# Developer-Zer0/GIF-synthesis-with-Discrete-Diffusion

Measured on NVIDIA B200. Metric: reverse_step_token_updates_per_sec, higher is better.
Workload: dtype f32

## Files before the change

### gif-synthesis-with-discrete-diffusion_b200/csrc/d3pm_ptx.cuh

```cuda
#pragma once

#include <cuda_runtime.h>
#include <stdint.h>

namespace d3pm {

__device__ __forceinline__ uint32_t smem_u32(const void* p) { return static_cast<uint32_t>(__cvta_generic_to_shared(p)); }

__device__ __forceinline__ void mbar_init(unsigned long long* bar, uint32_t count) {
  asm volatile("mbarrier.init.shared::cta.b64 [%0], %1;" ::"r"(smem_u32(bar)), "r"(count) : "memory");
}
__device__ __forceinline__ void fence_mbarrier_init() { asm volatile("fence.mbarrier_init.release.cluster;" ::: "memory"); }
__device__ __forceinline__ void mbar_expect_tx(unsigned long long* bar, uint32_t bytes) {
  asm volatile("mbarrier.arrive.expect_tx.shared::cta.b64 _, [%0], %1;" ::"r"(smem_u32(bar)), "r"(bytes) : "memory");
}
__device__ __forceinline__ void mbar_arrive(unsigned long long* bar) {
  asm volatile("mbarrier.arrive.shared::cta.b64 _, [%0];" ::"r"(smem_u32(bar)) : "memory");
}
__device__ __forceinline__ void mbar_arrive_remote(unsigned long long* bar, uint32_t cta) {
  uint32_t r;
  asm volatile("mapa.shared::cluster.u32 %0, %1, %2;" : "=r"(r) : "r"(smem_u32(bar)), "r"(cta));
  asm volatile("mbarrier.arrive.release.cluster.shared::cluster.b64 _, [%0];" ::"r"(r) : "memory");
}
__device__ __forceinline__ bool mbar_test(unsigned long long* bar, uint32_t parity) {
  uint32_t done;
  asm volatile(
      "{\n\t.reg .pred p;\n\t"
      "mbarrier.test_wait.parity.shared::cta.b64 p, [%1], %2;\n\t"
      "selp.u32 %0, 1, 0, p;\n\t}"
      : "=r"(done)
      : "r"(smem_u32(bar)), "r"(parity)
      : "memory");
  return done != 0;
}
__device__ __forceinline__ void mbar_wait(unsigned long long* bar, uint32_t parity) {
  asm volatile(
      "{\n\t.reg .pred p;\n\t"
      "WAIT_%=:\n\t"
      "mbarrier.try_wait.parity.shared::cta.b64 p, [%0], %1, %2;\n\t"
      "@p bra DONE_%=;\n\t"
      "bra WAIT_%=;\n\t"
      "DONE_%=:\n\t}"
      ::"r"(smem_u32(bar)), "r"(parity), "r"(0x989680)
      : "memory");
}
__device__ __forceinline__ void mbar_wait_spin(unsigned long long* bar, uint32_t parity) {
  const uint32_t addr = smem_u32(bar);
  uint32_t done;
  do {
    asm volatile(
        "{\n\t.reg .pred p;\n\t"
        "mbarrier.try_wait.parity.shared::cta.b64 p, [%1], %2;\n\t"
        "selp.u32 %0, 1, 0, p;\n\t}"
        : "=r"(done)
        : "r"(addr), "r"(parity)
        : "memory");
  } while (!done);
}
__device__ __forceinline__ void mbar_wait_cluster(unsigned long long* bar, uint32_t parity) {
  asm volatile(
      "{\n\t.reg .pred p;\n\t"
      "WAIT_%=:\n\t"
      "mbarrier.try_wait.parity.acquire.cluster.shared::cta.b64 p, [%0], %1, %2;\n\t"
      "@p bra DONE_%=;\n\t"
      "bra WAIT_%=;\n\t"
      "DONE_%=:\n\t}"
      ::"r"(smem_u32(bar)), "r"(parity), "r"(0x989680)
      : "memory");
}

__device__ __forceinline__ void tma_load(void* dst, const void* src, uint32_t bytes, unsigned long long* bar) {
  asm volatile(
      "cp.async.bulk.shared::cluster.global.mbarrier::complete_tx::bytes [%0], [%1], %2, [%3];"
      ::"r"(smem_u32(dst)), "l"(src), "r"(bytes), "r"(smem_u32(bar))
      : "memory");
}
__device__ __forceinline__ void fence_proxy_async() { asm volatile("fence.proxy.async.shared::cta;" ::: "memory"); }

__device__ __forceinline__ void tc_fence_before() { asm volatile("tcgen05.fence::before_thread_sync;" ::: "memory"); }
__device__ __forceinline__ void tc_fence_after() { asm volatile("tcgen05.fence::after_thread_sync;" ::: "memory"); }
__device__ __forceinline__ void tc_commit(unsigned long long* bar) {
  asm volatile("tcgen05.commit.cta_group::1.mbarrier::arrive::one.shared::cluster.b64 [%0];" ::"r"(smem_u32(bar)) : "memory");
}
__device__ __forceinline__ void tc_commit_pair(unsigned long long* bar) {
  asm volatile("tcgen05.commit.cta_group::2.mbarrier::arrive::one.shared::cluster.multicast::cluster.b64 [%0], %1;" ::"r"(smem_u32(bar)),
               "h"(static_cast<unsigned short>(3))
               : "memory");
}
constexpr uint32_t idesc_tf32(int M, int N) {
  return (1u << 4) | (2u << 7) | (2u << 10) | ((static_cast<uint32_t>(N) >> 3) << 17) | ((static_cast<uint32_t>(M) >> 4) << 24);
}
__device__ __forceinline__ void tc_mma_tf32(uint32_t d_tmem, uint64_t a_desc, uint64_t b_desc, uint32_t idesc, uint32_t accumulate) {
  asm volatile(
      "{\n\t.reg .pred p;\n\t"
      "setp.ne.b32 p, %4, 0;\n\t"
      "tcgen05.mma.cta_group::1.kind::tf32 [%0], %1, %2, %3, p;\n\t}"
      ::"r"(d_tmem), "l"(a_desc), "l"(b_desc), "r"(idesc), "r"(accumulate)
      : "memory");
}
__device__ __forceinline__ void tc_mma_tf32_pair(uint32_t d_tmem, uint64_t a_desc, uint64_t b_desc, uint32_t idesc, uint32_t accumulate) {
  asm volatile(
      "{\n\t.reg .pred p;\n\t"
      "setp.ne.b32 p, %4, 0;\n\t"
      "tcgen05.mma.cta_group::2.kind::tf32 [%0], %1, %2, %3, p;\n\t}"
      ::"r"(d_tmem), "l"(a_desc), "l"(b_desc), "r"(idesc), "r"(accumulate)
      : "memory");
}
__device__ __forceinline__ uint64_t smem_desc(uint32_t addr) {
  return static_cast<uint64_t>((addr >> 4) & 0x3fffu) | (static_cast<uint64_t>(1024 >> 4) << 32) | (1ull << 46) | (2ull << 61);
}

template <int CTAS, int NCOLS>
__device__ __forceinline__ void tmem_alloc(uint32_t* slot) {
  static_assert(CTAS == 1 || CTAS == 2, "cta_group::1 or ::2");
  if constexpr (CTAS == 2)
    asm volatile("tcgen05.alloc.cta_group::2.sync.aligned.shared::cta.b32 [%0], %1;" ::"r"(smem_u32(slot)), "n"(NCOLS) : "memory");
  else
    asm volatile("tcgen05.alloc.cta_group::1.sync.aligned.shared::cta.b32 [%0], %1;" ::"r"(smem_u32(slot)), "n"(NCOLS) : "memory");
}
template <int CTAS>
__device__ __forceinline__ void tmem_relinquish() {
  static_assert(CTAS == 1 || CTAS == 2, "cta_group::1 or ::2");
  if constexpr (CTAS == 2) asm volatile("tcgen05.relinquish_alloc_permit.cta_group::2.sync.aligned;" ::: "memory");
  else asm volatile("tcgen05.relinquish_alloc_permit.cta_group::1.sync.aligned;" ::: "memory");
}
template <int CTAS, int NCOLS>
__device__ __forceinline__ void tmem_dealloc(uint32_t taddr) {
  static_assert(CTAS == 1 || CTAS == 2, "cta_group::1 or ::2");
  if constexpr (CTAS == 2) asm volatile("tcgen05.dealloc.cta_group::2.sync.aligned.b32 %0, %1;" ::"r"(taddr), "n"(NCOLS) : "memory");
  else asm volatile("tcgen05.dealloc.cta_group::1.sync.aligned.b32 %0, %1;" ::"r"(taddr), "n"(NCOLS) : "memory");
}
__device__ __forceinline__ void tmem_ld16(uint32_t taddr, uint32_t (&v)[16]) {
  asm volatile(
      "tcgen05.ld.sync.aligned.32x32b.x16.b32 "
      "{%0, %1, %2, %3, %4, %5, %6, %7, %8, %9, %10, %11, %12, %13, %14, %15}, [%16];"
      : "=r"(v[0]), "=r"(v[1]), "=r"(v[2]), "=r"(v[3]), "=r"(v[4]), "=r"(v[5]), "=r"(v[6]), "=r"(v[7]), "=r"(v[8]),
        "=r"(v[9]), "=r"(v[10]), "=r"(v[11]), "=r"(v[12]), "=r"(v[13]), "=r"(v[14]), "=r"(v[15])
      : "r"(taddr)
      : "memory");
}
__device__ __forceinline__ void tmem_ld32(uint32_t taddr, uint32_t (&v)[32]) {
  asm volatile(
      "tcgen05.ld.sync.aligned.32x32b.x32.b32 "
      "{%0, %1, %2, %3, %4, %5, %6, %7, %8, %9, %10, %11, %12, %13, %14, %15, "
      "%16, %17, %18, %19, %20, %21, %22, %23, %24, %25, %26, %27, %28, %29, %30, %31}, [%32];"
      : "=r"(v[0]), "=r"(v[1]), "=r"(v[2]), "=r"(v[3]), "=r"(v[4]), "=r"(v[5]), "=r"(v[6]), "=r"(v[7]), "=r"(v[8]),
        "=r"(v[9]), "=r"(v[10]), "=r"(v[11]), "=r"(v[12]), "=r"(v[13]), "=r"(v[14]), "=r"(v[15]), "=r"(v[16]),
        "=r"(v[17]), "=r"(v[18]), "=r"(v[19]), "=r"(v[20]), "=r"(v[21]), "=r"(v[22]), "=r"(v[23]), "=r"(v[24]),
        "=r"(v[25]), "=r"(v[26]), "=r"(v[27]), "=r"(v[28]), "=r"(v[29]), "=r"(v[30]), "=r"(v[31])
      : "r"(taddr)
      : "memory");
}
__device__ __forceinline__ void tmem_ld_wait() { asm volatile("tcgen05.wait::ld.sync.aligned;" ::: "memory"); }

__device__ __forceinline__ uint32_t cluster_ctarank() {
  uint32_t r;
  asm volatile("mov.u32 %0, %%cluster_ctarank;" : "=r"(r));
  return r;
}
__device__ __forceinline__ void cluster_sync() {
  asm volatile("barrier.cluster.arrive.release;" ::: "memory");
  asm volatile("barrier.cluster.wait.acquire;" ::: "memory");
}

}
```

### gif-synthesis-with-discrete-diffusion_b200/csrc/d3pm_step_stream.cuh

```cuda
#pragma once

#include <cuda_fp16.h>

#include <type_traits>

#include "d3pm_host.h"
#include "d3pm_ptx.cuh"
#include "d3pm_step_rows.cuh"

namespace d3pm {

constexpr int kGroupThreads = 128;
constexpr int kGroupWarps = kGroupThreads / 32;
constexpr int kGroupsPerCta = 4;
constexpr int kStreamThreads = kGroupThreads * kGroupsPerCta;
constexpr int kCandPerRow = 30;
constexpr float kStreamThin = 8.0f;
constexpr float kRedoThin = 16.0f;
constexpr int kCoefSmemRows = 256;
struct RowInfo {
  float A, Bc, Pj, PK, accept;
  uint32_t j;
  int32_t rel;
  int32_t pad;
};

template <int NP, int CPT, bool HAS_U>
struct StreamShape {
  static_assert(CPT == 8 || (CPT == 16 && !HAS_U), "64 classes per thread only fit in registers without the second tensor");
  static constexpr int K = 1024 * NP;
  static constexpr int GT = 256 * NP / CPT;
  static constexpr int NW = GT / 32;
  static constexpr int NG = kStreamThreads / GT;
  static constexpr int SB = 128 / NG;
  static constexpr int RC = 8192 / NG;
  static constexpr int PS = 128 / GT;
  static constexpr int NCALL = CPT / 2;
  static_assert(GT >= 32 && GT <= 128 && NG <= 16, "unsupported group shape");
};

template <int NP, int CPT, bool HAS_U>
struct __align__(128) GroupSmem {
  using Sh = StreamShape<NP, CPT, HAS_U>;
  float c[1024 * NP];
  float u[HAS_U ? 1024 * NP : 4];
  alignas(16) float red[3][6 * 4];
  unsigned long long full;
  unsigned long long keys[4];
  uint32_t redo_cnt;
  uint32_t pad;
  RowInfo info[Sh::SB];
  uint32_t cand_cnt[Sh::SB];
  uint32_t cand_k[Sh::SB][kCandPerRow];
  float cand_p[Sh::SB][kCandPerRow];
  int32_t redo[Sh::RC];
};

__device__ __forceinline__ void group_bar(int id) {
  asm volatile("bar.sync %0, %1;" ::"r"(id), "n"(kGroupThreads) : "memory");
}
struct GroupSync {
  int id;
  __device__ __forceinline__ void operator()() const { group_bar(id); }
};
template <int NW>
struct StreamSync {
  int id;
  __device__ __forceinline__ void operator()() const {
    if (NW == 1) __syncwarp();
    else asm volatile("bar.sync %0, %1;" ::"r"(id), "n"(32 * NW) : "memory");
  }
};
__device__ __forceinline__ float4 lds4(const float* p) { return *reinterpret_cast<const float4*>(p); }
template <int LD>
struct LogitType {
  static constexpr uint32_t kBytes = LD == D3PM_LOGITS_F32 ? 4u : 2u;
  static __device__ __forceinline__ float2 widen(uint32_t pair) {
    if constexpr (LD == D3PM_LOGITS_BF16) {
      return make_float2(__uint_as_float(pair << 16), __uint_as_float(pair & 0xffff0000u));
    } else {
      return __half22float2(*reinterpret_cast<const __half2*>(&pair));
    }
  }
  static __device__ __forceinline__ void chunk(const float* stage, int q, float2& lo, float2& hi) {
    if constexpr (LD == D3PM_LOGITS_F32) {
      const float4 a = lds4(stage + 4 * q);
      lo = make_float2(a.x, a.y), hi = make_float2(a.z, a.w);
    } else {
      const uint2 raw = *reinterpret_cast<const uint2*>(reinterpret_cast<const unsigned char*>(stage) + 8 * q);
      lo = widen(raw.x), hi = widen(raw.y);
    }
  }
  static __device__ __forceinline__ float one(const float* stage, uint32_t k) {
    if constexpr (LD == D3PM_LOGITS_F32) {
      return stage[k];
    } else {
      const uint32_t h = reinterpret_cast<const unsigned short*>(stage)[k];
      if constexpr (LD == D3PM_LOGITS_BF16) return __uint_as_float(h << 16);
      else return __half2float(__ushort_as_half(static_cast<unsigned short>(h)));
    }
  }
  static __device__ __forceinline__ const void* row(const float* base, unsigned long long elements) {
    return reinterpret_cast<const unsigned char*>(base) + elements * kBytes;
  }
};
template <int NW>
__device__ __forceinline__ float4 lds_warps(const float* p, float neutral) {
  if (NW == 4) return lds4(p);
  const float2 a = *reinterpret_cast<const float2*>(p);
  return make_float4(a.x, a.y, neutral, neutral);
}
template <int NW, int NV, typename Sync>
__device__ __forceinline__ void stream_max_sum(float (&m)[NV], float (&s)[NV], float* scratch, Sync sync) {
  const int lane = threadIdx.x & 31, warp = (threadIdx.x >> 5) & (NW - 1);
#pragma unroll
  for (int v = 0; v < NV; ++v) {
    const float mw = warp_max(m[v]);
    const float mw2 = to_log2_units(mw);
    const float sw = warp_sum(s[v] * ex2(to_log2_units(m[v]) - mw2));
    if (NW == 1) {
      m[v] = mw, s[v] = sw;
    } else if (lane == 0) {
      scratch[(3 * v) * 4 + warp] = mw;
      scratch[(3 * v + 1) * 4 + warp] = mw2;
      scratch[(3 * v + 2) * 4 + warp] = sw;
    }
  }
  sync();
  if constexpr (NW > 1) {
#pragma unroll
  for (int v = 0; v < NV; ++v) {
    const float4 mw = lds_warps<NW>(scratch + (3 * v) * 4, -CUDART_INF_F), mw2 = lds_warps<NW>(scratch + (3 * v + 1) * 4, 0.f);
    const float4 sw = lds_warps<NW>(scratch + (3 * v + 2) * 4, 0.f);
    if (NW == 4) {
      const float M = fmaxf(fmaxf(mw.x, mw.y), fmaxf(mw.z, mw.w));
      const float M2 = to_log2_units(M);
      m[v] = M;
      s[v] = fmaf(sw.x, ex2(mw2.x - M2), fmaf(sw.y, ex2(mw2.y - M2), fmaf(sw.z, ex2(mw2.z - M2), sw.w * ex2(mw2.w - M2))));
    } else {
      const float M = fmaxf(mw.x, mw.y);
      const float M2 = to_log2_units(M);
      m[v] = M;
      s[v] = fmaf(sw.x, ex2(mw2.x - M2), sw.y * ex2(mw2.y - M2));
    }
  }
  }
}

__device__ __forceinline__ float warp_min(float x) {
  float m;
  asm volatile("redux.sync.min.f32 %0, %1, 0xffffffff;" : "=f"(m) : "f"(x));
  return m;
}

template <int NW, int NV, typename Sync>
__device__ __forceinline__ void stream_max(float* mx, float* scratch, Sync sync) {
  const int lane = threadIdx.x & 31, warp = (threadIdx.x >> 5) & (NW - 1);
#pragma unroll
  for (int v = 0; v < NV; ++v) {
    const float a = warp_max(mx[v]);
    if (NW == 1) mx[v] = a;
    else if (lane == 0) scratch[v * 4 + warp] = a;
  }
  sync();
  if constexpr (NW > 1) {
#pragma unroll
  for (int v = 0; v < NV; ++v) {
    const float4 a = lds_warps<NW>(scratch + v * 4, -CUDART_INF_F);
    mx[v] = fmaxf(fmaxf(a.x, a.y), fmaxf(a.z, a.w));
  }
  }
}

template <int NW, int NV, typename Sync>
__device__ __forceinline__ void stream_sum(float (&s)[NV], float* scratch, Sync sync) {
  const int lane = threadIdx.x & 31, warp = (threadIdx.x >> 5) & (NW - 1);
#pragma unroll
  for (int v = 0; v < NV; ++v) {
    const float sw = warp_sum(s[v]);
    if (NW == 1) s[v] = sw;
    else if (lane == 0) scratch[v * 4 + warp] = sw;
  }
  sync();
  if constexpr (NW > 1) {
#pragma unroll
  for (int v = 0; v < NV; ++v) {
    const float4 a = lds_warps<NW>(scratch + v * 4, 0.f);
    s[v] = (a.x + a.y) + (a.z + a.w);
  }
  }
}

template <int NW, typename Sync>
__device__ __forceinline__ unsigned long long stream_max_u64(unsigned long long key, unsigned long long* scratch, Sync sync) {
  const int lane = threadIdx.x & 31, warp = (threadIdx.x >> 5) & (NW - 1);
  key = warp_max_u64(key);
  if (NW == 1) {
    sync();
    return key;
  }
  if (lane == 0) scratch[warp] = key;
  sync();
  unsigned long long best = scratch[0];
#pragma unroll
  for (int w = 1; w < NW; ++w) best = scratch[w] > best ? scratch[w] : best;
  return best;
}

template <int NP, int CPT, bool HAS_U>
__device__ __noinline__ void score_batch(GroupSmem<NP, CPT, HAS_U>& S, int nslots, const ParamNoiseStream& rng, const StepParams& p, int G,
                                         int first_row) {
  using Sh = StreamShape<NP, CPT, HAS_U>;
  constexpr uint32_t K = 1024u * NP;
  const int lane = threadIdx.x & 31, warp = (threadIdx.x >> 5) & (Sh::NW - 1);
  const int sub = lane & 15;
  for (int slot = 2 * warp + (lane >> 4); slot - (lane >> 4) < nslots; slot += 2 * Sh::NW) {
    unsigned long long key = 0ull;
    float lp = 0.f;
    const bool live = slot < nslots;
    RowInfo ri;
    ri.accept = 0.f, ri.rel = 0;
    uint32_t cnt = 0;
    if (live) {
      ri = S.info[slot];
      cnt = S.cand_cnt[slot];
      const uint32_t n = cnt < static_cast<uint32_t>(kCandPerRow) ? cnt : static_cast<uint32_t>(kCandPerRow);
      const uint64_t grow = static_cast<uint64_t>(p.row_offset + (first_row + ri.rel * G));
      for (uint32_t item = static_cast<uint32_t>(sub); item < n + 2u; item += 16u) {
        uint32_t k = 0;
        float P = 0.f;
        bool have = false;
        if (item < n) {
          k = S.cand_k[slot][item];
          const float pe = fminf(fmaxf(S.cand_p[slot][item], kPFloor), 1.0f);
          P = fmaf(pe, ri.A, ri.Bc);
          have = (k != ri.j);
        } else if (item == n) {
          k = K, P = ri.PK, have = true;
        } else if (ri.j != K) {
          k = ri.j, P = ri.Pj, have = true;
        }
        if (have) {
          const float lpk = log_prob_clamped(P);
          const float sc = lpk + gumbel_from_uniform(uniform_from_draw(rng.draw(k, grow)));
          const unsigned long long kk = pack_key(sc, k);
          if (kk > key) key = kk, lp = lpk;
        }
      }
    }
    const unsigned long long mine = key;
#pragma unroll
    for (int o = 8; o > 0; o >>= 1) {
      const unsigned long long other = __shfl_xor_sync(0xffffffffu, key, o);
      key = other > key ? other : key;
    }
    const bool accepted = live && cnt <= static_cast<uint32_t>(kCandPerRow) && key_score(key) >= ri.accept;
    if (live && sub == 0) {
      if (accepted) {
        p.x_prev[first_row + ri.rel * G] = key_class(key);
      } else {
        S.redo[atomicAdd(&S.redo_cnt, 1u)] = ri.rel;
      }
      S.cand_cnt[slot] = 0;
    }
    if (p.winner_post != nullptr && accepted && mine == key && mine != 0ull) p.winner_post[first_row + ri.rel * G] = lp;
  }
}

template <int NP, int CPT, bool HAS_U, bool RECON, int LD = D3PM_LOGITS_F32>
__global__ void __launch_bounds__(kStreamThreads, 1) step_stream_kernel(const __grid_constant__ StepParams p) {
  extern __shared__ __align__(128) unsigned char smem_raw[];
  using Sh = StreamShape<NP, CPT, HAS_U>;
  using Smem = GroupSmem<NP, CPT, HAS_U>;
  constexpr int K = Sh::K, GT = Sh::GT, NW = Sh::NW, NG = Sh::NG, PS = Sh::PS, NCALL = Sh::NCALL;
  constexpr int NC = CPT;
  using LT = LogitType<LD>;
  constexpr uint32_t kRowBytes = K * LT::kBytes;
  uint32_t tid;
  asm volatile("mov.u32 %0, %%tid.x;" : "=r"(tid));
  const int g = tid / GT;
  const int tg = tid % GT;
  Smem& S = reinterpret_cast<Smem*>(smem_raw)[g];
  const StreamSync<NW> sync{g + 1};
  const int G = static_cast<int>(gridDim.x) * NG;
  const int first_row = g * static_cast<int>(gridDim.x) + static_cast<int>(blockIdx.x);
  const int rows = static_cast<int>(p.rows);
  const uint32_t pitch = static_cast<uint32_t>(p.pitch_logits);
  const bool exact_mode = (p.sample_mode == D3PM_SAMPLE_PHILOX_EXACT);
  if (tg == 0) {
    mbar_init(&S.full, 1);
    fence_mbarrier_init();
    S.redo_cnt = 0;
    if (!exact_mode && first_row < rows) {
      const unsigned long long at = static_cast<unsigned long long>(static_cast<uint32_t>(first_row)) * pitch;
      mbar_expect_tx(&S.full, HAS_U ? 2 * kRowBytes : kRowBytes);
      tma_load(S.c, LT::row(p.logits_c, at), kRowBytes, &S.full);
      if (HAS_U) tma_load(S.u, LT::row(p.logits_u, at), kRowBytes, &S.full);
    }
  }
  float* coef_s = reinterpret_cast<float*>(smem_raw + sizeof(Smem) * NG);
  const bool coef_in_smem = p.T <= kCoefSmemRows;
  if (coef_in_smem) {
    for (int i = tid; i < p.T * 16; i += kStreamThreads)
      coef_s[i] = __ldg(p.coef_table + static_cast<size_t>(i >> 4) * D3PM_COEF_STRIDE + (i & 15));
  }
  const ParamNoiseStream rng(NoiseKeysParam(p.keys), p.offset);
  const float thin_c = p.thin_factor > 0.f ? p.thin_factor : kStreamThin;
  for (int i = tg; i < Sh::SB; i += GT) S.cand_cnt[i] = 0;
  __syncthreads();

  auto issue_row = [&](int row) {
    const unsigned long long at = static_cast<unsigned long long>(static_cast<uint32_t>(row)) * pitch;
    fence_proxy_async();
    mbar_expect_tx(&S.full, HAS_U ? 2 * kRowBytes : kRowBytes);
    tma_load(S.c, LT::row(p.logits_c, at), kRowBytes, &S.full);
    if (HAS_U) tma_load(S.u, LT::row(p.logits_u, at), kRowBytes, &S.full);
  };
  auto slot_lo = [](int c) { return (c / PS) * 2 * PS + (c % PS); };

  uint32_t phase = 0;
  uint32_t status_bits = 0;
#ifdef D3PM_STREAM_TIMING
  auto now_ns = [] { unsigned long long v; asm volatile("mov.u64 %0, %%globaltimer;" : "=l"(v)); return v; };
  const unsigned long long tm_start = now_ns();
  unsigned long long tm_main = 0;
  uint32_t tm_rows = 0, tm_redo = 0;
#endif

  auto process_row = [&](auto exact_c, int row, int next_row, uint32_t j, int tt, int slot, int rel) {
    constexpr bool exact = decltype(exact_c)::value;
    const bool masked = (j == static_cast<uint32_t>(K));
    mbar_wait_spin(&S.full, phase);
    phase ^= 1u;

    float2 x[NC][2], z[HAS_U ? NC : 1][2];
#pragma unroll
    for (int i = 0; i < NC; ++i) {
      const int q = GT * i + tg;
      LT::chunk(S.c, q, x[i][0], x[i][1]);
      if (HAS_U) LT::chunk(S.u, q, z[i][0], z[i][1]);
    }
    auto e_of = [&](int i, int h) -> float2& {
      if constexpr (HAS_U) return z[i][h];
      else return x[i][h];
    };
    const float xj = masked ? 0.f : LT::one(S.c, j);
    const float zj = (HAS_U && !masked) ? LT::one(S.u, j) : 0.f;

    float am[2] = {0.f, 0.f};
    if (HAS_U) {
      am[0] = fmaxf(fmaxf(fabsf(x[0][0].x), fabsf(x[0][0].y)), fmaxf(fabsf(x[0][1].x), fabsf(x[0][1].y)));
      am[1] = fmaxf(fmaxf(fabsf(z[0][0].x), fabsf(z[0][0].y)), fmaxf(fabsf(z[0][1].x), fabsf(z[0][1].y)));
    }
#pragma unroll
    for (int i = 1; i < NC; ++i) {
      if (HAS_U)
        am[0] = fmaxf(fmaxf(am[0], fabsf(x[i][0].x)), fmaxf(fabsf(x[i][0].y), fmaxf(fabsf(x[i][1].x), fabsf(x[i][1].y))));
      if (HAS_U)
        am[1] = fmaxf(fmaxf(am[1], fabsf(z[i][0].x)), fmaxf(fabsf(z[i][0].y), fmaxf(fabsf(z[i][1].x), fabsf(z[i][1].y))));
    }
    if (HAS_U) stream_max<NW, 2>(am, S.red[0], sync);
    else sync();
    if (!exact && tg == 0 && next_row >= 0) issue_row(next_row);

    const uint64_t grow = static_cast<uint64_t>(p.row_offset + row);

    float My2, rSy, r, yj;
    const float2 l2e = make_float2(kLog2e, kLog2e);
    if (HAS_U) {
      const float gs = p.guidance_scale, og = 1.0f - gs;
      const float2 gs2 = make_float2(gs, gs), og2 = make_float2(og, og);
      float my = -CUDART_INF_F;
      constexpr float kLnK = NP == 4 ? 8.3178f : (NP == 2 ? 7.6247f : 6.9315f);
      constexpr float kSafeAbs = 0.5f * (69.99f - kLnK);
      const bool no_clamp = (am[0] <= kSafeAbs) && (am[1] <= kSafeAbs) && (fabsf(gs) * am[0] + fabsf(og) * am[1] <= 160.0f);
      if (no_clamp) {
#pragma unroll
        for (int i = 0; i < NC; ++i)
#pragma unroll
          for (int h = 0; h < 2; ++h) {
            const float2 y = __ffma2_rn(gs2, x[i][h], __fmul2_rn(og2, z[i][h]));
            x[i][h] = y;
            my = fmaxf(my, fmaxf(y.x, y.y));
          }
        yj = fmaf(gs, xj, og * zj);
      } else {
        float mx[2], s[2];
        mx[0] = fmaxf(fmaxf(x[0][0].x, x[0][0].y), fmaxf(x[0][1].x, x[0][1].y));
        mx[1] = fmaxf(fmaxf(z[0][0].x, z[0][0].y), fmaxf(z[0][1].x, z[0][1].y));
#pragma unroll
        for (int i = 1; i < NC; ++i) {
          mx[0] = fmaxf(fmaxf(mx[0], x[i][0].x), fmaxf(x[i][0].y, fmaxf(x[i][1].x, x[i][1].y)));
          mx[1] = fmaxf(fmaxf(mx[1], z[i][0].x), fmaxf(z[i][0].y, fmaxf(z[i][1].x, z[i][1].y)));
        }
        stream_max<NW, 2>(mx, S.red[2], sync);
        mx[0] = fmaxf(mx[0], -3.0e38f), mx[1] = fmaxf(mx[1], -3.0e38f);
        {
          const float mc2 = to_log2_units(mx[0]), mu2 = to_log2_units(mx[1]);
          const float2 nmc = make_float2(-mc2, -mc2), nmu = make_float2(-mu2, -mu2);
          float2 sc[2] = {make_float2(0.f, 0.f), make_float2(0.f, 0.f)}, su[2] = {sc[0], sc[0]};
#pragma unroll
          for (int i = 0; i < NC; ++i)
#pragma unroll
            for (int h = 0; h < 2; ++h) {
              const float2 ac = __ffma2_rn(x[i][h], l2e, nmc), au = __ffma2_rn(z[i][h], l2e, nmu);
              sc[h] = __fadd2_rn(sc[h], make_float2(ex2(ac.x), ex2(ac.y)));
              su[h] = __fadd2_rn(su[h], make_float2(ex2(au.x), ex2(au.y)));
            }
          s[0] = (sc[0].x + sc[0].y) + (sc[1].x + sc[1].y);
          s[1] = (su[0].x + su[0].y) + (su[1].x + su[1].y);
        }
        stream_sum<NW, 2>(s, S.red[2] + 2 * 4, sync);
        const float lnSc = ln_rel_sum(mx[0], s[0]), lnSu = ln_rel_sum(mx[1], s[1]);
        const float ta = kClampLo + lnSc, tb = kClampLo + lnSu;
        const float C = fmaf(-gs, lnSc, -og * lnSu);
        const float2 nMc = make_float2(-mx[0], -mx[0]), nMu = make_float2(-mx[1], -mx[1]), C2 = make_float2(C, C);
#pragma unroll
        for (int i = 0; i < NC; ++i)
#pragma unroll
          for (int h = 0; h < 2; ++h) {
            float2 a = __fadd2_rn(x[i][h], nMc), b = __fadd2_rn(z[i][h], nMu);
            a.x = fmaxf(a.x, ta), a.y = fmaxf(a.y, ta);
            b.x = fmaxf(b.x, tb), b.y = fmaxf(b.y, tb);
            const float2 y = __ffma2_rn(gs2, a, __ffma2_rn(og2, b, C2));
            x[i][h] = y;
            my = fmaxf(my, fmaxf(y.x, y.y));
          }
        yj = fmaf(gs, fmaxf(xj - mx[0], ta), fmaf(og, fmaxf(zj - mx[1], tb), C));
      }
      const float my2 = to_log2_units(my);
      {
        const float2 nmy = make_float2(-my2, -my2);
        float2 sy[2] = {make_float2(0.f, 0.f), make_float2(0.f, 0.f)};
#pragma unroll
        for (int i = 0; i < NC; ++i)
#pragma unroll
          for (int h = 0; h < 2; ++h) {
            const float2 ay = __ffma2_rn(x[i][h], l2e, nmy);
            const float2 ey = make_float2(ex2(ay.x), ex2(ay.y));
            e_of(i, h) = ey;
            sy[h] = __fadd2_rn(sy[h], ey);
          }
        float mm[1] = {my}, ss[1] = {(sy[0].x + sy[0].y) + (sy[1].x + sy[1].y)};
        stream_max_sum<NW, 1>(mm, ss, S.red[1], sync);
        My2 = to_log2_units(mm[0]);
        rSy = __fdividef(1.0f, ss[0]);
      }
      r = ex2(my2 - My2) * rSy;
    } else {
      float mx[1];
      mx[0] = fmaxf(fmaxf(x[0][0].x, x[0][0].y), fmaxf(x[0][1].x, x[0][1].y));
#pragma unroll
      for (int i = 1; i < NC; ++i) mx[0] = fmaxf(fmaxf(mx[0], x[i][0].x), fmaxf(x[i][0].y, fmaxf(x[i][1].x, x[i][1].y)));
      mx[0] = fmaxf(mx[0], -3.0e38f);
      const float mc2 = to_log2_units(mx[0]);
      const float2 nmc = make_float2(-mc2, -mc2);
      float2 sc[2] = {make_float2(0.f, 0.f), make_float2(0.f, 0.f)};
#pragma unroll
      for (int i = 0; i < NC; ++i)
#pragma unroll
        for (int h = 0; h < 2; ++h) {
          const float2 ac = __ffma2_rn(x[i][h], l2e, nmc);
          const float2 ec = make_float2(ex2(ac.x), ex2(ac.y));
          e_of(i, h) = ec;
          sc[h] = __fadd2_rn(sc[h], ec);
        }
      float ss[1] = {(sc[0].x + sc[0].y) + (sc[1].x + sc[1].y)};
      stream_max_sum<NW, 1>(mx, ss, S.red[1], sync);
      My2 = to_log2_units(mx[0]);
      rSy = __fdividef(1.0f, ss[0]);
      r = ex2(mc2 - My2) * rSy;
      yj = xj;
    }
    const float pj = masked ? 0.f : fminf(fmaxf(ex2(fmaf(yj, kLog2e, -My2)) * rSy, kPFloor), 1.0f);
    RowCoef cf;
    if (coef_in_smem) {
      const float* crow = coef_s + tt * 16 + (masked ? 0 : 8);
      cf = row_coef_from(lds4(crow), lds4(crow + 4), masked);
    } else {
      cf = load_row_coef(p.coef_table, tt, masked);
    }
    RowMath rm;
    if (RECON) {
      rm.init_recon(masked ? 0.f : pj, masked ? static_cast<uint32_t>(K) + 1u : j);
      if (tg == 0 && p.score != nullptr) p.score[row] = fminf(fmaxf(rSy, kPFloor), 1.0f);
    } else {
      rm.init(cf, masked, pj, j, K);
    }

    if constexpr (!exact) {
      const ThinRule thin(rm, thin_c);
      const float thrA = r * thin.scaleA, nthrB = -thin.thrB;
      const float2 tA2 = make_float2(thrA, thrA);
      if (tg == 0) {
        RowInfo ri;
        ri.A = rm.A, ri.Bc = rm.Bc, ri.Pj = rm.Pj, ri.PK = rm.PK, ri.accept = thin.accept;
        ri.j = j, ri.rel = rel, ri.pad = 0;
        S.info[slot] = ri;
      }
#pragma unroll
      for (int c0 = 0; c0 < NCALL; c0 += 4) {
        uint4 cws[4];
#pragma unroll
        for (int c = 0; c < 4; ++c) cws[c] = rng.coarse(ParamNoiseStream::coarse_call_of_chunk(GT * slot_lo(c0 + c) + tg), grow);
#pragma unroll
        for (int c = 0; c < 4; ++c) {
          const int lo = slot_lo(c0 + c);
          const uint32_t w4[4] = {cws[c].x, cws[c].y, cws[c].z, cws[c].w};
          float slack = -4.0f;
#pragma unroll
          for (int w = 0; w < 4; ++w) {
            const float2 nf = make_float2(__uint_as_float(__byte_perm(w4[w], 0xbf80u, 0x5410)),
                                          __uint_as_float(__byte_perm(w4[w], 0xbf80u, 0x5432)));
            const float2 d = __ffma2_rn(e_of(lo + (w >> 1) * PS, w & 1), tA2, nf);
            slack = fmaxf(slack, fmaxf(d.x, d.y));
          }
          if (slack >= nthrB) {
#pragma unroll
            for (int w = 0; w < 4; ++w)
#pragma unroll
              for (int hl = 0; hl < 2; ++hl) {
                const float2 ee = e_of(lo + (w >> 1) * PS, w & 1);
                const float e = hl ? ee.y : ee.x;
                const uint32_t h16 = hl ? (w4[w] >> 16) : (w4[w] & 0xffffu);
                const float nf = __uint_as_float(0xbf800000u | h16);
                if (fmaf(e, thrA, nf) >= nthrB) {
                  const uint32_t pos = atomicAdd(&S.cand_cnt[slot], 1u);
                  if (pos < static_cast<uint32_t>(kCandPerRow)) {
                    S.cand_k[slot][pos] = 4u * (GT * (lo + (w >> 1) * PS) + tg) + 2u * (w & 1) + hl;
                    S.cand_p[slot][pos] = e * r;
                  }
                }
              }
          }
        }
      }
      return;
    } else {
    unsigned long long best = 0ull;
    float best_lp = 0.f;
    bool settled = false;
    if (!exact_mode) {
      const ThinRule thin2(rm, (p.thin_factor > 0.f && p.thin_factor < 0.01f) ? p.thin_factor : kRedoThin);
      const float thrA = r * thin2.scaleA;
      const float2 tA2 = make_float2(thrA, thrA), tB2 = make_float2(thin2.thrB, thin2.thrB);
#pragma unroll
      for (int c = 0; c < NCALL; ++c) {
        const int lo = slot_lo(c);
        const uint4 cw = rng.coarse(ParamNoiseStream::coarse_call_of_chunk(GT * lo + tg), grow);
        const uint32_t w4[4] = {cw.x, cw.y, cw.z, cw.w};
        uint32_t hits = 0;
        float ev[8];
#pragma unroll
        for (int w = 0; w < 4; ++w) {
          const float2 ee = e_of(lo + (w >> 1) * PS, w & 1);
          ev[2 * w] = ee.x, ev[2 * w + 1] = ee.y;
          const float2 nf = make_float2(__uint_as_float(__byte_perm(w4[w], 0xbf80u, 0x5410)),
                                        __uint_as_float(__byte_perm(w4[w], 0xbf80u, 0x5432)));
          const float2 d = __ffma2_rn(ee, tA2, __fadd2_rn(tB2, nf));
          hits |= (d.x >= 0.0f ? 1u : 0u) << (2 * w);
          hits |= (d.y >= 0.0f ? 1u : 0u) << (2 * w + 1);
        }
        while (hits != 0) {
          const int b = __ffs(hits) - 1;
          hits &= hits - 1;
          float e = 0.f;
#pragma unroll
          for (int q = 0; q < 8; ++q) e = (b == q) ? ev[q] : e;
          const uint32_t k = 4u * (GT * (lo + (b >> 2) * PS) + tg) + static_cast<uint32_t>(b & 3);
          if (k != j) {
            const float lpk = rm.post_of(k, e, r);
            const unsigned long long key = pack_key(lpk + gumbel_from_uniform(uniform_from_draw(rng.draw(k, grow))), k);
            if (key > best) best = key, best_lp = lpk;
          }
        }
      }
      if (tg == 0) {
        const float lpk = rm.post_mask();
        const unsigned long long key = pack_key(lpk + gumbel_from_uniform(uniform_from_draw(rng.draw(K, grow))), K);
        if (key > best) best = key, best_lp = lpk;
      }
      if (tg == GT - 1 && !masked) {
        const float lpk = rm.post_self();
        const unsigned long long key = pack_key(lpk + gumbel_from_uniform(uniform_from_draw(rng.draw(j, grow))), j);
        if (key > best) best = key, best_lp = lpk;
      }
      const unsigned long long mine = best;
      best = stream_max_u64<NW>(best, S.keys, sync);
      settled = key_score(best) >= thin2.accept;
      if (settled) {
        if (p.winner_post != nullptr && mine == best) p.winner_post[row] = best_lp;
      } else {
        best = 0ull;
        sync();
      }
    }
    if (!settled) {
#pragma unroll
      for (int i = 0; i < NC; ++i) {
        const float2 a = e_of(i, 0), b = e_of(i, 1);
        *reinterpret_cast<float4*>(S.c + 4 * (GT * i + tg)) = make_float4(a.x, a.y, b.x, b.y);
      }
#pragma unroll 1
      for (int i = 0; i < NC; ++i) {
        const uint32_t q = static_cast<uint32_t>(GT) * i + tg;
        const float4 e4 = lds4(S.c + 4 * q);
        const float ev[4] = {e4.x, e4.y, e4.z, e4.w};
        const uint4 cw = rng.coarse(ParamNoiseStream::coarse_call_of_chunk(q), grow);
        const uint4 fw = rng.fine(q >> 2, grow);
#pragma unroll
        for (int e = 0; e < 4; ++e) {
          const uint32_t k = 4u * q + e;
          const uint32_t mdraw =
              (ParamNoiseStream::half_of(cw, (((q >> 7) & 1u) << 2) | e) << 7) | ParamNoiseStream::low7_of(fw, ((q & 3u) << 2) | e);
          const float lpk = rm.post_of(k, ev[e], r);
          const unsigned long long key = pack_key(lpk + gumbel_from_uniform(uniform_from_draw(mdraw)), k);
          if (key > best) best = key, best_lp = lpk;
        }
      }
      if (tg == 0) {
        const float lpk = rm.post_mask();
        const unsigned long long key = pack_key(lpk + gumbel_from_uniform(uniform_from_draw(rng.draw(K, grow))), K);
        if (key > best) best = key, best_lp = lpk;
      }
      const unsigned long long mine = best;
      best = stream_max_u64<NW>(best, S.keys, sync);
      if (p.winner_post != nullptr && mine == best) p.winner_post[row] = best_lp;
    }
    if (tg == 0) {
      p.x_prev[row] = key_class(best);
      if (next_row >= 0) issue_row(next_row);
    }
    }
  };

  const int N = p.N;
  auto token_of = [&](int r_) { return static_cast<long long>(p.x_t[r_]); };
  auto time_of = [&](int b_) { return static_cast<long long>(p.t[b_]); };
  auto checked = [&](long long tt, long long jj, int& t_cur, uint32_t& j_cur) {
    if (static_cast<unsigned long long>(tt) >= static_cast<unsigned long long>(p.T)) {
      status_bits |= D3PM_STATUS_BAD_T;
      tt = tt < 0 ? 0 : p.T - 1;
    }
    if (static_cast<unsigned long long>(jj) > static_cast<unsigned long long>(K)) {
      status_bits |= D3PM_STATUS_BAD_TOKEN;
      jj = K;
    }
    t_cur = static_cast<int>(tt), j_cur = static_cast<uint32_t>(jj);
    asm volatile("" : "+r"(t_cur), "+r"(j_cur) : : "memory");
  };
  if (!exact_mode) {
    const int stepB = G / N, stepR = G % N;
    int vb = first_row / N, vr = first_row % N;
    int row = first_row < rows ? first_row : -1;
    long long jj = 0, tt = 0;
    if (row >= 0) {
      jj = token_of(row);
      tt = time_of(vb);
    }
    int it = 0, in_batch = 0;
    while (row >= 0) {
      int t_cur;
      uint32_t j_cur;
      checked(tt, jj, t_cur, j_cur);
      const int next = row + G < rows ? row + G : -1;
      vb += stepB, vr += stepR;
      if (vr >= N) vr -= N, ++vb;
      if (next >= 0) {
        jj = token_of(next);
        tt = time_of(vb);
      }
      process_row(std::false_type{}, row, next, j_cur, t_cur, in_batch, it);
#ifdef D3PM_STREAM_TIMING
      ++tm_rows;
#endif
      row = next;
      ++it;
      if (++in_batch == Sh::SB || row < 0) {
        sync();
        score_batch<NP, CPT, HAS_U>(S, in_batch, rng, p, G, first_row);
        sync();
        in_batch = 0;
      }
    }
  }
#ifdef D3PM_STREAM_TIMING
  tm_main = now_ns();
#endif
  {
    const uint32_t n2 = exact_mode ? (first_row < rows ? static_cast<uint32_t>((rows - first_row + G - 1) / G) : 0u) : S.redo_cnt;
    auto row_at = [&](uint32_t i) { return first_row + (exact_mode ? static_cast<int>(i) : S.redo[i]) * G; };
    if (n2 > 0) {
      if (!exact_mode) status_bits |= D3PM_STATUS_FALLBACK;
      int row = row_at(0);
      if (tg == 0) issue_row(row);
      long long jj = token_of(row), tt = time_of(row / N);
      for (uint32_t i = 0; i < n2; ++i) {
        int t_cur;
        uint32_t j_cur;
        checked(tt, jj, t_cur, j_cur);
        const int next = (i + 1 < n2) ? row_at(i + 1) : -1;
        if (next >= 0) {
          jj = token_of(next);
          tt = time_of(next / N);
        }
        process_row(std::true_type{}, row, next, j_cur, t_cur, 0, 0);
#ifdef D3PM_STREAM_TIMING
        ++tm_redo;
#endif
        row = next;
      }
    }
  }
#ifdef D3PM_STREAM_TIMING
  if (tg == 0 && p.status != nullptr) {
    const unsigned long long tm_end = now_ns();
    uint32_t* o = p.status + 8 * (blockIdx.x * NG + g);
    uint32_t smid;
    asm volatile("mov.u32 %0, %%smid;" : "=r"(smid));
    o[0] = static_cast<uint32_t>(tm_start), o[1] = static_cast<uint32_t>(tm_start >> 32);
    o[2] = static_cast<uint32_t>(tm_main - tm_start), o[3] = static_cast<uint32_t>(tm_end - tm_start);
    o[4] = tm_rows, o[5] = tm_redo, o[6] = smid, o[7] = 0;
  }
#else
  if (status_bits != 0 && tg == 0 && p.status != nullptr) atomicOr(p.status, status_bits);
#endif
}

constexpr long long kStreamMinRows = 1024;

inline bool stream_kernel_supports(const StepParams& p) {
  if (p.sample_mode != D3PM_SAMPLE_PHILOX && p.sample_mode != D3PM_SAMPLE_PHILOX_EXACT) return false;
  if (p.post != nullptr || p.recon != nullptr || p.gap != nullptr || p.x_prev == nullptr) return false;
  if (p.sharpen != nullptr || (p.score != nullptr && p.sample_from != D3PM_FROM_RECON)) return false;
  if (p.K != 1024 && p.K != 2048 && p.K != 4096) return false;
  if (p.pitch_logits >= (1LL << 32)) return false;
  if (p.logits_dtype != D3PM_LOGITS_F32 && (p.sample_from == D3PM_FROM_RECON || p.pitch_logits % 8 != 0)) return false;
  return true;
}

inline long long stream_kernel_max_rows() { return 8192LL * host::sm_count(); }

template <int NP, int CPT, bool HAS_U, bool RECON, int LD>
int launch_step_stream_r(const StepParams& p, cudaStream_t s) {
  using Sh = StreamShape<NP, CPT, HAS_U>;
  const int sms = host::sm_count();
  if (sms == 0) return D3PM_ERR_CUDA;
  const size_t smem = sizeof(GroupSmem<NP, CPT, HAS_U>) * Sh::NG + kCoefSmemRows * 16 * sizeof(float);
  auto kern = step_stream_kernel<NP, CPT, HAS_U, RECON, LD>;
  if (cudaFuncSetAttribute(kern, cudaFuncAttributeMaxDynamicSharedMemorySize, static_cast<int>(smem)) != cudaSuccess)
    return D3PM_ERR_CUDA;
  kern<<<static_cast<unsigned>(sms), kStreamThreads, smem, s>>>(p);
  return D3PM_OK;
}

template <int NP, int CPT, bool HAS_U>
int launch_step_stream_t(const StepParams& p, cudaStream_t s) {
  if (p.logits_dtype == D3PM_LOGITS_F16)
    return p.sample_from == D3PM_FROM_RECON ? D3PM_ERR_UNSUPPORTED : launch_step_stream_r<NP, CPT, HAS_U, false, D3PM_LOGITS_F16>(p, s);
  if (p.logits_dtype == D3PM_LOGITS_BF16)
    return p.sample_from == D3PM_FROM_RECON ? D3PM_ERR_UNSUPPORTED : launch_step_stream_r<NP, CPT, HAS_U, false, D3PM_LOGITS_BF16>(p, s);
  return p.sample_from == D3PM_FROM_RECON ? launch_step_stream_r<NP, CPT, HAS_U, true, D3PM_LOGITS_F32>(p, s)
                                          : launch_step_stream_r<NP, CPT, HAS_U, false, D3PM_LOGITS_F32>(p, s);
}

inline int launch_step_stream(const StepParams& p, cudaStream_t s) {
  const bool has_u = p.logits_u != nullptr;
  switch (p.K) {
    case 1024: return has_u ? launch_step_stream_t<1, 8, true>(p, s) : launch_step_stream_t<1, 8, false>(p, s);
    case 2048: return has_u ? launch_step_stream_t<2, 8, true>(p, s) : launch_step_stream_t<2, 16, false>(p, s);
    case 4096: return has_u ? launch_step_stream_t<4, 8, true>(p, s) : launch_step_stream_t<4, 16, false>(p, s);
    default: return D3PM_ERR_UNSUPPORTED;
  }
}

}
```

Baseline: 204.8 million.

## Issue next-row TMA early via an empty mbarrier instead of after reduction sync

Adds an 'empty' mbarrier that every warp arrives on once it has read the current row's staged logits. The group's leader warp waits on it and then immediately issues the TMA for the next row, rather than waiting until after the max-reduction block sync. The goal is to overlap the next row's load with the reduction and sampling math, shortening the wait on the full barrier. It also adds timing instrumentation that only runs under a debug macro, and it relies on all warps having finished their shared-memory reads before the buffer is overwritten.

```diff
diff --git a/gif-synthesis-with-discrete-diffusion_b200/csrc/d3pm_ptx.cuh b/gif-synthesis-with-discrete-diffusion_b200/csrc/d3pm_ptx.cuh
--- a/gif-synthesis-with-discrete-diffusion_b200/csrc/d3pm_ptx.cuh
+++ b/gif-synthesis-with-discrete-diffusion_b200/csrc/d3pm_ptx.cuh
@@ -54,6 +54,24 @@
         "selp.u32 %0, 1, 0, p;\n\t}"
         : "=r"(done)
         : "r"(addr), "r"(parity)
+        : "memory");
+  } while (!done);
+}
+__device__ __forceinline__ uint64_t mbar_arrive_state(unsigned long long* bar) {
+  uint64_t state;
+  asm volatile("mbarrier.arrive.shared::cta.b64 %0, [%1];" : "=l"(state) : "r"(smem_u32(bar)) : "memory");
+  return state;
+}
+__device__ __forceinline__ void mbar_wait_state_spin(unsigned long long* bar, uint64_t state) {
+  const uint32_t addr = smem_u32(bar);
+  uint32_t done;
+  do {
+    asm volatile(
+        "{\n\t.reg .pred p;\n\t"
+        "mbarrier.try_wait.shared::cta.b64 p, [%1], %2;\n\t"
+        "selp.u32 %0, 1, 0, p;\n\t}"
+        : "=r"(done)
+        : "r"(addr), "l"(state)
         : "memory");
   } while (!done);
 }
diff --git a/gif-synthesis-with-discrete-diffusion_b200/csrc/d3pm_step_stream.cuh b/gif-synthesis-with-discrete-diffusion_b200/csrc/d3pm_step_stream.cuh
--- a/gif-synthesis-with-discrete-diffusion_b200/csrc/d3pm_step_stream.cuh
+++ b/gif-synthesis-with-discrete-diffusion_b200/csrc/d3pm_step_stream.cuh
@@ -46,7 +46,8 @@
   float u[HAS_U ? 1024 * NP : 4];
   alignas(16) float red[3][6 * 4];
   unsigned long long full;
-  unsigned long long keys[4];
+  unsigned long long empty;
+  unsigned long long keys[Sh::NW];
   uint32_t redo_cnt;
   uint32_t pad;
   RowInfo info[Sh::SB];
@@ -71,6 +72,16 @@
     else asm volatile("bar.sync %0, %1;" ::"r"(id), "n"(32 * NW) : "memory");
   }
 };
+template <int NW>
+__device__ __forceinline__ bool stage_released(unsigned long long* empty) {
+  __syncwarp();
+  if ((threadIdx.x & 31) != 0) return false;
+  if constexpr (NW == 1) return true;
+  const uint64_t state = mbar_arrive_state(empty);
+  if (((threadIdx.x >> 5) & (NW - 1)) != 0) return false;
+  mbar_wait_state_spin(empty, state);
+  return true;
+}
 __device__ __forceinline__ float4 lds4(const float* p) { return *reinterpret_cast<const float4*>(p); }
 template <int LD>
 struct LogitType {
@@ -289,6 +300,7 @@
   const bool exact_mode = (p.sample_mode == D3PM_SAMPLE_PHILOX_EXACT);
   if (tg == 0) {
     mbar_init(&S.full, 1);
+    if (NW > 1) mbar_init(&S.empty, NW);
     fence_mbarrier_init();
     S.redo_cnt = 0;
     if (!exact_mode && first_row < rows) {
@@ -323,14 +335,22 @@
 #ifdef D3PM_STREAM_TIMING
   auto now_ns = [] { unsigned long long v; asm volatile("mov.u64 %0, %%globaltimer;" : "=l"(v)); return v; };
   const unsigned long long tm_start = now_ns();
+  const long long tm_clk0 = clock64();
   unsigned long long tm_main = 0;
+  long long tm_clk_main = 0, tm_wait_clk = 0;
   uint32_t tm_rows = 0, tm_redo = 0;
 #endif
 
   auto process_row = [&](auto exact_c, int row, int next_row, uint32_t j, int tt, int slot, int rel) {
     constexpr bool exact = decltype(exact_c)::value;
     const bool masked = (j == static_cast<uint32_t>(K));
+#ifdef D3PM_STREAM_TIMING
+    const long long tw0 = clock64();
+#endif
     mbar_wait_spin(&S.full, phase);
+#ifdef D3PM_STREAM_TIMING
+    if (!exact) tm_wait_clk += clock64() - tw0;
+#endif
     phase ^= 1u;
 
     float2 x[NC][2], z[HAS_U ? NC : 1][2];
@@ -346,6 +366,9 @@
     };
     const float xj = masked ? 0.f : LT::one(S.c, j);
     const float zj = (HAS_U && !masked) ? LT::one(S.u, j) : 0.f;
+    if constexpr (!exact) {
+      if (stage_released<NW>(&S.empty) && next_row >= 0) issue_row(next_row);
+    }
 
     float am[2] = {0.f, 0.f};
     if (HAS_U) {
@@ -361,7 +384,6 @@
     }
     if (HAS_U) stream_max<NW, 2>(am, S.red[0], sync);
     else sync();
-    if (!exact && tg == 0 && next_row >= 0) issue_row(next_row);
 
     const uint64_t grow = static_cast<uint64_t>(p.row_offset + row);
 
@@ -686,6 +708,7 @@
   }
 #ifdef D3PM_STREAM_TIMING
   tm_main = now_ns();
+  tm_clk_main = clock64() - tm_clk0;
 #endif
   {
     const uint32_t n2 = exact_mode ? (first_row < rows ? static_cast<uint32_t>((rows - first_row + G - 1) / G) : 0u) : S.redo_cnt;
@@ -720,7 +743,8 @@
     asm volatile("mov.u32 %0, %%smid;" : "=r"(smid));
     o[0] = static_cast<uint32_t>(tm_start), o[1] = static_cast<uint32_t>(tm_start >> 32);
     o[2] = static_cast<uint32_t>(tm_main - tm_start), o[3] = static_cast<uint32_t>(tm_end - tm_start);
-    o[4] = tm_rows, o[5] = tm_redo, o[6] = smid, o[7] = 0;
+    const double ns_per_clk = tm_clk_main > 0 ? static_cast<double>(tm_main - tm_start) / static_cast<double>(tm_clk_main) : 0.0;
+    o[4] = tm_rows, o[5] = tm_redo, o[6] = smid, o[7] = static_cast<uint32_t>(static_cast<double>(tm_wait_clk) * ns_per_clk);
   }
 #else
   if (status_bits != 0 && tg == 0 && p.status != nullptr) atomicOr(p.status, status_bits);
```

After: 204.2 million (median of 6 runs). Within noise of the previous version (-0.3%).
